# ultralytics/yolov5

Measured on NVIDIA H100. Metric: images/sec @640 (forward + NMS), higher is better.
Workload: dtype bf16

## Files before the change

### yolov5_b200/csrc/conv_gemm.cu

```cuda
#include <cstdio>
#include <cstdlib>
#include <cstring>
#include <mutex>

#include "../../include/y5b200.h"
#include "common.cuh"
#include "host_util.h"
#include "wgmma.cuh"

namespace y5 {

constexpr int kBlockM = 128;
constexpr int kConsumers = 2;
constexpr int kConsumerThreads = 128 * kConsumers;
constexpr int kThreads = 128 + kConsumerThreads;
constexpr int kMaxStages = 8;
constexpr int kHeadN = 128;

enum AMode { A_LINEAR = 0, A_IM2COL = 1, A_PATCH = 2 };

struct ConvParams {
    int M, N;
    int num_m_tiles;
    int num_m_super, num_n_tiles;
    int kh, kw, c_chunks;
    int block_k;
    int a_mode;
    int Ho, Wo, HoWo, stride, pad_h, pad_w;
    int tw, th, tiles_x, tiles_y;
    int b_grouped;
    int patch_pw;
    int cluster_n;
    uint32_t stg_bytes;
    uint32_t b_sub_bytes;
    float rcp_per_img, rcp_tiles_x, rcp_HoWo, rcp_Wo;
    int a_stages, b_stages;
    uint32_t a_sub_bytes, a_stage_bytes, b_stage_bytes;
    int is_bf16, act;
    const float* bias;
    int bias_n;
    void* out;
    int out_pitch;
    const void* res;
    int res_pitch;
    void* raw;
    void* z;
    int na, no, nc, nx, z_rows, z_row0;
    float det_stride;
    float anchor_wh[8];
};

struct SmemLayout {
    uint32_t off_a, off_b, off_out, off_bias, off_bars, total;
};

__host__ __device__ inline SmemLayout smem_layout(int epi, int no, int bias_n, int a_stages, int b_stages, uint32_t a_bytes,
                                                   uint32_t b_bytes, uint32_t stg_bytes) {
    SmemLayout L;
    uint32_t o = 0;
    L.off_a = o;
    o += a_stages * a_bytes;
    L.off_b = o;
    o += b_stages * b_bytes;
    o = (o + 1023) & ~1023u;
    L.off_out = o;
    if (epi == 1) o += 4 * ((kBlockM * no * 2 + 1023) & ~1023u);
    else o += stg_bytes;
    L.off_bias = o;
    o += ((bias_n + 3) & ~3) * 4;
    o = (o + 7) & ~7u;
    L.off_bars = o;
    o += 4 * kMaxStages * 8;
    L.total = o;
    return L;
}

__device__ __forceinline__ int fdiv(int n, int d, float rd) {
    if (n >= (1 << 23)) return n / d;
    int q = __float2int_rz(__int2float_rz(n) * rd);
    const int r = n - q * d;
    if (r >= d) ++q;
    else if (r < 0) --q;
    return q;
}

template <int BLOCK_N, int EPI, int MT, bool OPT>
__global__ void __launch_bounds__(kThreads, 1)
conv_gemm_kernel(const __grid_constant__ CUtensorMap tmA, const __grid_constant__ CUtensorMap tmB, const ConvParams p) {
    static_assert(MT * BLOCK_N <= 256, "accumulators: at most 128 fp32 registers per consumer thread");
    constexpr int kAcc = BLOCK_N / 2;

    extern __shared__ __align__(1024) uint8_t smem_raw[];
    uint8_t* smem = reinterpret_cast<uint8_t*>((reinterpret_cast<uintptr_t>(smem_raw) + 1023) & ~uintptr_t(1023));
    const SmemLayout L = smem_layout(EPI, p.no, p.bias_n, p.a_stages, p.b_stages, p.a_stage_bytes, p.b_stage_bytes, p.stg_bytes);
    uint8_t* sA = smem + L.off_a;
    uint8_t* sB = smem + L.off_b;
    float* sBias = reinterpret_cast<float*>(smem + L.off_bias);
    uint64_t* a_full = reinterpret_cast<uint64_t*>(smem + L.off_bars);
    uint64_t* a_empty = a_full + kMaxStages;
    uint64_t* b_full = a_empty + kMaxStages;
    uint64_t* b_empty = b_full + kMaxStages;

    const int warp = threadIdx.x >> 5;
    const int lane = threadIdx.x & 31;
    const int csize = OPT ? static_cast<int>(cluster_nctarank()) : 1;
    const uint32_t crank = OPT ? cluster_ctarank() : 0u;

    if (threadIdx.x == 0) {
        tma_prefetch_desc(&tmA);
        tma_prefetch_desc(&tmB);
        for (int s = 0; s < kMaxStages; ++s) {
            mbar_init(&a_full[s], 1);
            mbar_init(&a_empty[s], kConsumers);
            mbar_init(&b_full[s], 1);
            mbar_init(&b_empty[s], kConsumers * csize);
        }
        fence_barrier_init();
    }
    if (threadIdx.x >= 128)
        for (int i = threadIdx.x - 128; i < p.bias_n; i += kConsumerThreads) {
            const float b = i < p.N ? __ldg(p.bias + i) : 0.0f;
            sBias[i] = (EPI == 0 && p.act) ? 0.5f * b : b;
        }
    __syncthreads();
    if (csize > 1) cluster_sync_all();
    griddep_wait();
    griddep_launch_dependents();

    const int nn = p.num_n_tiles;
    const int num_tiles = ((p.num_m_super + csize - 1) / csize) * nn;
    const int tile0 = blockIdx.x / csize, tile_step = gridDim.x / csize;
    const uint32_t row_bytes = p.block_k * 2;
    const bool patch = p.a_mode == A_PATCH;
    const bool wide = OPT && p.patch_pw > 0;
    const int grp = wide ? p.kh * p.kw : (patch ? p.kh : 1);
    const int num_groups = wide ? p.c_chunks : (patch ? p.c_chunks * p.kw : p.kh * p.kw * p.c_chunks);

    if (warp < 4) {
        setmaxnreg_dec<56>();
    }
    if (warp == 0) {
        int as = 0, bs = 0;
        uint32_t aph = 0, bph = 0;
        for (int tile = tile0; tile < num_tiles; tile += tile_step) {
            const int ms = (tile / nn) * csize + static_cast<int>(crank);
            const int n0 = (tile - (tile / nn) * nn) * BLOCK_N;
            int img[MT], y0[MT], x0[MT];
#pragma unroll
            for (int mi = 0; mi < MT; ++mi) {
                const int mt = ms * MT + mi;
                img[mi] = y0[mi] = x0[mi] = 0;
                if (p.a_mode == A_IM2COL) {
                    const int m0 = mt * kBlockM;
                    img[mi] = fdiv(m0, p.HoWo, p.rcp_HoWo);
                    const int rem = m0 - img[mi] * p.HoWo;
                    const int oy = fdiv(rem, p.Wo, p.rcp_Wo);
                    y0[mi] = oy * p.stride - p.pad_h;
                    x0[mi] = (rem - oy * p.Wo) * p.stride - p.pad_w;
                } else if (patch) {
                    const int per_img = p.tiles_x * p.tiles_y;
                    img[mi] = fdiv(mt, per_img, p.rcp_per_img);
                    const int rem = mt - img[mi] * per_img;
                    const int ty = fdiv(rem, p.tiles_x, p.rcp_tiles_x);
                    y0[mi] = ty * p.th - p.pad_h;
                    x0[mi] = (rem - ty * p.tiles_x) * p.tw - p.pad_w;
                }
            }
            auto issue_group = [&](int cc, int s, int r0) {
                mbar_wait(&a_empty[as], aph ^ 1);
// ... 16 lines not shown
                for (int j = 0; j < grp; ++j) {
                    const int r = patch ? j : r0;
                    const int kb = wide ? j * p.c_chunks + cc : (r * p.kw + s) * p.c_chunks + cc;
                    const bool stage_first = !p.b_grouped || j == 0, stage_last = !p.b_grouped || j == grp - 1;
                    if (stage_first) mbar_wait(&b_empty[bs], bph ^ 1);
                    if (elect_one()) {
                        if (stage_first) mbar_arrive_expect_tx(&b_full[bs], p.b_stage_bytes);
                        uint8_t* b_dst = sB + bs * p.b_stage_bytes + (p.b_grouped ? j * p.b_sub_bytes : 0u);
                        if (csize == 1) tma_load_2d(&tmB, &b_full[bs], b_dst, kb * p.block_k, n0);
                        else {
                            const int slice_rows = BLOCK_N / csize;
                            tma_load_2d_mcast(&tmB, &b_full[bs], b_dst + crank * slice_rows * row_bytes, kb * p.block_k,
                                              n0 + static_cast<int>(crank) * slice_rows, static_cast<uint16_t>((1u << csize) - 1u));
                        }
                    }
                    __syncwarp();
                    if (stage_last && ++bs == p.b_stages) { bs = 0; bph ^= 1; }
                }
            };
            if (wide) {
                for (int cc = 0; cc < p.c_chunks; ++cc) issue_group(cc, 0, 0);
            } else if (patch) {
                for (int cc = 0; cc < p.c_chunks; ++cc)
                    for (int s = 0; s < p.kw; ++s) issue_group(cc, s, 0);
            } else {
                for (int r = 0; r < p.kh; ++r)
                    for (int s = 0; s < p.kw; ++s)
                        for (int cc = 0; cc < p.c_chunks; ++cc) issue_group(cc, s, r);
            }
        }
    } else if (warp >= 4) {
    setmaxnreg_inc<224>();
    const int wg = (warp >> 2) - 1;
    const int ct = threadIdx.x - 128;
    const int wrow = wg * 64 + (warp & 3) * 16 + (lane >> 2);
    const int ccol = 2 * (lane & 3);
    const bool signal = (threadIdx.x & 127) == 0;
    const bool bf16 = p.is_bf16 != 0;
    const uint32_t dhi = gmma_desc_hi(row_bytes);
    const uint32_t a_hi = wide ? (dhi & ~0x3FFFu) | (((static_cast<uint32_t>(p.patch_pw) * row_bytes) >> 4) & 0x3FFFu) : dhi;
    const uint32_t a_base = gmma_desc_lo(smem_u32(sA) + (wide ? wg * 8 * p.patch_pw : wg * 64) * row_bytes), b_base = gmma_desc_lo(smem_u32(sB));
    const uint32_t row16 = row_bytes >> 4;
    const uint32_t a_stage16 = p.a_stage_bytes >> 4, b_stage16 = p.b_stage_bytes >> 4, a_sub16 = p.a_sub_bytes >> 4;
    const uint32_t b_sub16 = p.b_sub_bytes >> 4;
    const uint32_t a_shift16 = patch ? (p.tw * row_bytes) >> 4 : 0;
    const int k_steps = p.block_k / 16;
    const int per_img = p.tiles_x * p.tiles_y;
    const int tw_shift = patch ? __ffs(p.tw) - 1 : 0;
    int as = 0, bs = 0, head_set = 0;
    uint32_t aph = 0, bph = 0;
    float acc[MT][kAcc];
#pragma unroll
    for (int mi = 0; mi < MT; ++mi)
#pragma unroll
        for (int i = 0; i < kAcc; ++i) acc[mi][i] = 0.0f;

    for (int tile = tile0; tile < num_tiles; tile += tile_step) {
        const int ms = (tile / nn) * csize + static_cast<int>(crank);
        const int nt = tile - (tile / nn) * nn;
        const int n0 = nt * BLOCK_N;
        for (int g = 0; g < num_groups; ++g) {
            mbar_wait(&a_full[as], aph);
            const uint32_t a_stage_lo = a_base + as * a_stage16;
            uint32_t a_lo = a_stage_lo;
            for (int j = 0; j < grp; ++j) {
                if (wide) {
                    const int tr = j / p.kw, ts = j - tr * p.kw;
                    a_lo = a_stage_lo + (tr * p.patch_pw + ts) * row16;
                }
                const bool stage_first = !p.b_grouped || j == 0, stage_last = !p.b_grouped || j == grp - 1;
                if (stage_first) mbar_wait(&b_full[bs], bph);
                const uint32_t b_lo = b_base + bs * b_stage16 + (p.b_grouped ? j * b_sub16 : 0u);
#pragma unroll
                for (int mi = 0; mi < MT; ++mi) fence_regs(acc[mi]);
                wgmma_fence();
#pragma unroll
                for (int k = 0; k < 4; ++k) {
                    if (k < k_steps) {
                        const uint32_t scale_d = (g | j | k) != 0 ? 1u : 0u;
#pragma unroll
                        for (int mi = 0; mi < MT; ++mi) {
                            const uint64_t da = gmma_desc(a_lo + mi * a_sub16 + 2 * k, a_hi), db = gmma_desc(b_lo + 2 * k, dhi);
                            if (bf16) Wgmma<BLOCK_N>::template run<true, 0, 0>(acc[mi], da, db, scale_d);
                            else Wgmma<BLOCK_N>::template run<false, 0, 0>(acc[mi], da, db, scale_d);
                        }
                    }
                }
                wgmma_commit();
                wgmma_wait<0>();
#pragma unroll
                for (int mi = 0; mi < MT; ++mi) fence_regs(acc[mi]);
                if (stage_last) {
                    if (signal) {
                        if (csize == 1) mbar_arrive(&b_empty[bs]);
                        else
                            for (int r = 0; r < csize; ++r) mbar_arrive_cluster(mapa_u32(&b_empty[bs], static_cast<uint32_t>(r)));
                    }
                    if (++bs == p.b_stages) { bs = 0; bph ^= 1; }
                }
                a_lo += a_shift16;
            }
            if (signal) mbar_arrive(&a_empty[as]);
            if (++as == p.a_stages) { as = 0; aph ^= 1; }
        }

        if (EPI == 0) {
            const bool staged = OPT && p.stg_bytes != 0;
            const uint32_t stg_pitch = BLOCK_N * 2 + 16;
            uint8_t* stg = smem + L.off_out + wg * 64 * stg_pitch;
#pragma unroll
            for (int mi = 0; mi < MT; ++mi) {
                const int mt = ms * MT + mi;
                int img = 0, oy0 = 0, ox0 = 0;
                if (patch) {
                    img = fdiv(mt, per_img, p.rcp_per_img);
                    const int rem = mt - img * per_img;
                    const int tyi = fdiv(rem, p.tiles_x, p.rcp_tiles_x);
                    oy0 = tyi * p.th;
                    ox0 = (rem - tyi * p.tiles_x) * p.tw;
                }
                auto pixel_of = [&](int row) -> long long {
                    if (patch) {
                        const int oy = oy0 + (row >> tw_shift), ox = ox0 + (row & ((1 << tw_shift) - 1));
                        return (mt < p.num_m_tiles && oy < p.Ho && ox < p.Wo) ? static_cast<long long>(img) * p.HoWo + oy * p.Wo + ox : -1;
                    }
                    const long long m = static_cast<long long>(mt) * kBlockM + row;
                    return m < p.M ? m : -1;
                };
#pragma unroll
                for (int h = 0; h < 2; ++h) {
                    const int row = wrow + 8 * h;
                    const long long gpix = pixel_of(row);
                    if (gpix < 0 && !staged) continue;
                    uint16_t* op = reinterpret_cast<uint16_t*>(p.out) + gpix * p.out_pitch + n0 + ccol;
                    const uint16_t* rp = (p.res && gpix >= 0) ? reinterpret_cast<const uint16_t*>(p.res) + gpix * p.res_pitch + n0 + ccol : nullptr;
                    uint8_t* sp = stg + (row - wg * 64) * stg_pitch + ccol * 2;
#pragma unroll
                    for (int j = 0; j < BLOCK_N / 8; ++j) {
                        if (n0 + 8 * j >= p.N) continue;
                        const float2 b = *reinterpret_cast<const float2*>(sBias + n0 + 8 * j + ccol);
                        const float a0 = acc[mi][4 * j + 2 * h], a1 = acc[mi][4 * j + 2 * h + 1];
                        float f0, f1;
                        if (p.act) {
                            f0 = silu_from_half(fmaf(a0, 0.5f, b.x));
                            f1 = silu_from_half(fmaf(a1, 0.5f, b.y));
                        } else {
                            f0 = a0 + b.x;
                            f1 = a1 + b.y;
                        }
                        if (rp) {
                            const float2 t = unpack2(*reinterpret_cast<const uint32_t*>(rp + 8 * j), bf16);
                            f0 += t.x;
                            f1 += t.y;
                        }
                        if (staged) *reinterpret_cast<uint32_t*>(sp + 16 * j) = pack2(f0, f1, bf16);
                        else *reinterpret_cast<uint32_t*>(op + 8 * j) = pack2(f0, f1, bf16);
                    }
                }
                if (staged) {
                    named_bar_sync(2 + wg, 128);
                    constexpr int kSeg = BLOCK_N / 8;
                    for (int i = threadIdx.x & 127; i < 64 * kSeg; i += 128) {
                        const int lrow = i / kSeg, c = i - lrow * kSeg;
                        const long long gpix = pixel_of(wg * 64 + lrow);
                        if (gpix >= 0 && n0 + 8 * c < p.N)
                            *reinterpret_cast<uint4*>(reinterpret_cast<uint16_t*>(p.out) + gpix * p.out_pitch + n0 + 8 * c) =
                                *reinterpret_cast<const uint4*>(stg + lrow * stg_pitch + c * 16);
                    }
                    named_bar_sync(2 + wg, 128);
                }
            }
        } else {
            const uint32_t blk = (kBlockM * p.no * 2 + 1023) & ~1023u;
            const int set = head_set;
            head_set ^= 1;
            uint16_t* stage_raw = reinterpret_cast<uint16_t*>(smem + L.off_out + (2 * set) * blk);
            uint16_t* stage_z = reinterpret_cast<uint16_t*>(smem + L.off_out + (2 * set + 1) * blk);
            const int no = p.no;
            const int a = nt;
            const float aw = p.anchor_wh[a * 2], ah = p.anchor_wh[a * 2 + 1];
            const int m0 = ms * kBlockM;
            const int rows_here = min(kBlockM, p.M - m0);
#pragma unroll
            for (int h = 0; h < 2; ++h) {
                const int row = wrow + 8 * h;
                const int m = m0 + row;
                int gx = 0, gy = 0;
                if (m < p.M) { const int pix = m - fdiv(m, p.HoWo, p.rcp_HoWo) * p.HoWo; gy = fdiv(pix, p.nx, p.rcp_Wo); gx = pix - gy * p.nx; }
                const float fgx = static_cast<float>(gx) - 0.5f, fgy = static_cast<float>(gy) - 0.5f;
#pragma unroll
                for (int j = 0; j < BLOCK_N / 8; ++j) {
#pragma unroll
                    for (int e = 0; e < 2; ++e) {
                        const int o = 8 * j + ccol + e;
                        if (o >= no) continue;
                        const float x = acc[0][4 * j + 2 * h + e] + sBias[n0 + o];
                        float d = x;
                        if (o < 5 + p.nc) {
                            const float sg = sigmoid_f(x);
                            if (o == 0) d = (sg * 2.0f + fgx) * p.det_stride;
                            else if (o == 1) d = (sg * 2.0f + fgy) * p.det_stride;
                            else if (o == 2) { const float u = sg * 2.0f; d = u * u * aw; }
                            else if (o == 3) { const float u = sg * 2.0f; d = u * u * ah; }
                            else d = sg;
                        }
                        stage_raw[row * no + o] = pack1(x, bf16);
                        stage_z[row * no + o] = pack1(d, bf16);
                    }
                }
            }
            named_bar_sync(1, kConsumerThreads);
            const int b_lo = fdiv(m0, p.HoWo, p.rcp_HoWo), b_hi = fdiv(m0 + rows_here - 1, p.HoWo, p.rcp_HoWo);
            for (int b = b_lo; b <= b_hi; ++b) {
                const int r_lo = max(b * p.HoWo - m0, 0), r_hi = min((b + 1) * p.HoWo - m0, rows_here);
                const int pix_lo = m0 + r_lo - b * p.HoWo;
                const int n_el = (r_hi - r_lo) * no;
#pragma unroll
                for (int which = 0; which < 2; ++which) {
                    const long long dst_el = which == 0
                        ? ((static_cast<long long>(b) * p.na + a) * p.HoWo + pix_lo) * no
                        : (static_cast<long long>(b) * p.z_rows + p.z_row0 + static_cast<long long>(a) * p.HoWo + pix_lo) * no;
                    uint16_t* dst = reinterpret_cast<uint16_t*>(which == 0 ? p.raw : p.z) + dst_el;
                    const uint16_t* src = (which == 0 ? stage_raw : stage_z) + r_lo * no;
                    if ((((reinterpret_cast<uintptr_t>(dst) | reinterpret_cast<uintptr_t>(src)) & 15) == 0) && (n_el & 7) == 0) {
                        const uint4* s4 = reinterpret_cast<const uint4*>(src);
                        uint4* d4 = reinterpret_cast<uint4*>(dst);
                        for (int i = ct; i < n_el / 8; i += kConsumerThreads) d4[i] = s4[i];
                    } else {
                        for (int i = ct; i < n_el; i += kConsumerThreads) dst[i] = src[i];
                    }
                }
            }
        }
    }
    }
    if (csize > 1) cluster_sync_all();
}

__global__ void conv_direct_kernel(const uint16_t* __restrict__ in, long long xs, long long ys, long long ns, int B, int H,
                                   int W, int Cin, const uint16_t* __restrict__ w, int cin_pad, const float* __restrict__ bias,
                                   uint16_t* out, int out_pitch, int Cout, const uint16_t* res, int res_pitch, int kh, int kw,
                                   int stride, int pad_h, int pad_w, int Ho, int Wo, int act, int bf16) {
    const long long idx = static_cast<long long>(blockIdx.x) * blockDim.x + threadIdx.x;
    const long long total = static_cast<long long>(B) * Ho * Wo * Cout;
    if (idx >= total) return;
    const int n = static_cast<int>(idx % Cout);
    const long long m = idx / Cout;
    const int ox = static_cast<int>(m % Wo);
    const int oy = static_cast<int>((m / Wo) % Ho);
    const int b = static_cast<int>(m / (static_cast<long long>(Wo) * Ho));
    float acc = 0.0f;
    for (int r = 0; r < kh; ++r) {
        const int iy = oy * stride - pad_h + r;
        if (iy < 0 || iy >= H) continue;
        for (int s = 0; s < kw; ++s) {
            const int ix = ox * stride - pad_w + s;
            if (ix < 0 || ix >= W) continue;
            const uint16_t* ip = in + b * ns + iy * ys + ix * xs;
            const uint16_t* wp = w + (static_cast<long long>(n) * kh * kw + r * kw + s) * cin_pad;
            for (int c = 0; c < Cin; ++c) acc += unpack1(ip[c], bf16) * unpack1(wp[c], bf16);
        }
    }
    float x = acc + bias[n];
    if (act) x = x / (1.0f + expf(-x));
    if (res) x += unpack1(res[m * res_pitch + n], bf16);
    out[m * out_pitch + n] = pack1(x, bf16);
}

}

using namespace y5;

namespace {

int pick_block_k(int in_c) {
    return in_c > 16 ? 64 : 16;
}

void pick_tile(int out_c, int64_t m_tiles, int* block_n, int* mt) {
    const int64_t sms = sm_count();
    if (out_c <= 32) { *block_n = 32; *mt = 4; return; }
    if (out_c <= 64) { *block_n = 64; *mt = 2; return; }
    if (out_c <= 128) {
        *block_n = 128;
        *mt = ((m_tiles + 1) / 2) >= sms ? 2 : 1;
        return;
    }
    const int64_t tiles256 = m_tiles * ((out_c + 255) / 256);
    *block_n = (tiles256 >= 2 * sms && (out_c % 256 == 0 || out_c > 384)) ? 256 : 128;
    *mt = 1;
}

int pick_block_n(int out_c, int64_t m_rows) {
    int bn, mt;
    pick_tile(out_c, m_rows > 0 ? (m_rows + kBlockM - 1) / kBlockM : 1, &bn, &mt);
    return bn;
}

template <int BN, int EPI, int MT, bool OPT>
cudaError_t launch_conv(const CUtensorMap& a, const CUtensorMap& b, const ConvParams& p, int grid, int cluster, uint32_t smem,
                        cudaStream_t st) {
    const cudaError_t attr_err = ensure_dyn_smem(reinterpret_cast<const void*>(conv_gemm_kernel<BN, EPI, MT, OPT>), 227 * 1024);
    if (attr_err != cudaSuccess) return attr_err;
    count_launch();
    if (cluster == 1) return launch_pdl(conv_gemm_kernel<BN, EPI, MT, OPT>, dim3(grid), dim3(kThreads), smem, st, a, b, p);
    static const bool pdl = [] { const char* e = getenv("Y5_PDL"); return !(e && e[0] == '0'); }();
    cudaLaunchConfig_t cfg{};
    cfg.gridDim = dim3(grid);
    cfg.blockDim = dim3(kThreads);
    cfg.dynamicSmemBytes = smem;
    cfg.stream = st;
    cudaLaunchAttribute attr[2];
    attr[0].id = cudaLaunchAttributeClusterDimension;
    attr[0].val.clusterDim.x = cluster;
    attr[0].val.clusterDim.y = 1;
    attr[0].val.clusterDim.z = 1;
    attr[1].id = cudaLaunchAttributeProgrammaticStreamSerialization;
    attr[1].val.programmaticStreamSerializationAllowed = 1;
    cfg.attrs = attr;
    cfg.numAttrs = pdl ? 2 : 1;
    return cudaLaunchKernelEx(&cfg, conv_gemm_kernel<BN, EPI, MT, OPT>, a, b, p);
}

struct PlanCommon {
    CUtensorMap tmA, tmB;
    ConvParams p;
    int block_n, epi, mt, grid, cluster;
    uint32_t smem_bytes;
};

int finish_plan(PlanCommon& pc, int block_n, int epi, int mt, int cluster = 1) {
    ConvParams& p = pc.p;
    p.cluster_n = cluster;
    p.a_stage_bytes = mt * p.a_sub_bytes;
    if (p.patch_pw > 0) p.a_stage_bytes = static_cast<uint32_t>(p.th + p.kh - 1) * p.patch_pw * p.block_k * 2;
    p.num_m_super = (p.num_m_tiles + mt - 1) / mt;
    p.num_n_tiles = epi == 1 ? p.na : (p.N + block_n - 1) / block_n;
    p.bias_n = p.num_n_tiles * block_n;
    const uint32_t budget = 225 * 1024 - 1024;
    const bool patch = p.a_mode == A_PATCH;
    int a_st = 0, b_st = 0;
    if (!patch) {
        for (int s = kMaxStages; s >= 2; --s)
            if (smem_layout(epi, p.no, p.bias_n, s, s, p.a_stage_bytes, p.b_stage_bytes, p.stg_bytes).total <= budget) { a_st = b_st = s; break; }
    } else {
        const int b_min = p.b_grouped ? 2 : 3, b_max = p.b_grouped ? 4 : kMaxStages;
        for (int a = 3; a >= 2 && !a_st; --a)
            for (int b = b_max; b >= b_min; --b)
                if (smem_layout(epi, p.no, p.bias_n, a, b, p.a_stage_bytes, p.b_stage_bytes, p.stg_bytes).total <= budget) { a_st = a; b_st = b; break; }
    }
    if (a_st < 2 || b_st < 2) return set_error(Y5_E_UNSUPPORTED, "conv tile does not fit shared memory (block_n %d a %u b %u)", block_n,
                                                p.a_stage_bytes, p.b_stage_bytes);
    p.a_stages = a_st;
    p.b_stages = b_st;
    pc.smem_bytes = smem_layout(epi, p.no, p.bias_n, a_st, b_st, p.a_stage_bytes, p.b_stage_bytes, p.stg_bytes).total + 1024;
    pc.block_n = block_n;
    pc.epi = epi;
    pc.mt = mt;
    pc.cluster = cluster;
    const long long tiles = static_cast<long long>((p.num_m_super + cluster - 1) / cluster) * p.num_n_tiles;
    const int max_clusters = sm_count() / cluster;
    pc.grid = static_cast<int>(tiles < max_clusters ? tiles : max_clusters) * cluster;
    return 0;
}

int run_plan(const PlanCommon& pc, cudaStream_t st) {
    cudaError_t e = cudaErrorInvalidValue;
    const bool opt = pc.cluster > 1 || pc.p.patch_pw > 0 || pc.p.stg_bytes > 0;
    const int key = (opt ? 100000 : 0) + pc.epi * 10000 + pc.block_n * 10 + pc.mt;
    switch (key) {
        case 324: e = launch_conv<32, 0, 4, false>(pc.tmA, pc.tmB, pc.p, pc.grid, pc.cluster, pc.smem_bytes, st); break;
        case 642: e = launch_conv<64, 0, 2, false>(pc.tmA, pc.tmB, pc.p, pc.grid, pc.cluster, pc.smem_bytes, st); break;
        case 1281: e = launch_conv<128, 0, 1, false>(pc.tmA, pc.tmB, pc.p, pc.grid, pc.cluster, pc.smem_bytes, st); break;
        case 1282: e = launch_conv<128, 0, 2, false>(pc.tmA, pc.tmB, pc.p, pc.grid, pc.cluster, pc.smem_bytes, st); break;
        case 2561: e = launch_conv<256, 0, 1, false>(pc.tmA, pc.tmB, pc.p, pc.grid, pc.cluster, pc.smem_bytes, st); break;
        case 11281: e = launch_conv<kHeadN, 1, 1, false>(pc.tmA, pc.tmB, pc.p, pc.grid, pc.cluster, pc.smem_bytes, st); break;
        case 100324: e = launch_conv<32, 0, 4, true>(pc.tmA, pc.tmB, pc.p, pc.grid, pc.cluster, pc.smem_bytes, st); break;
        case 100642: e = launch_conv<64, 0, 2, true>(pc.tmA, pc.tmB, pc.p, pc.grid, pc.cluster, pc.smem_bytes, st); break;
        case 101281: e = launch_conv<128, 0, 1, true>(pc.tmA, pc.tmB, pc.p, pc.grid, pc.cluster, pc.smem_bytes, st); break;
        case 101282: e = launch_conv<128, 0, 2, true>(pc.tmA, pc.tmB, pc.p, pc.grid, pc.cluster, pc.smem_bytes, st); break;
        case 102561: e = launch_conv<256, 0, 1, true>(pc.tmA, pc.tmB, pc.p, pc.grid, pc.cluster, pc.smem_bytes, st); break;
        default: return set_error(Y5_E_UNSUPPORTED, "conv: no kernel for block_n %d mt %d epi %d", pc.block_n, pc.mt, pc.epi);
    }
    if (e != cudaSuccess) return set_error(int(e), "conv_gemm launch failed: %s", cudaGetErrorString(e));
    return 0;
}

bool aligned16(const void* p) { return (reinterpret_cast<uintptr_t>(p) & 15) == 0; }

struct Geo {
    int kh, kw, pad_h, pad_w, Ho, Wo;
    long long xs, ys, ns;
};
Geo geometry(const y5_conv_desc* d) {
    Geo g;
    g.kh = d->ksize;
    g.kw = d->kw ? d->kw : d->ksize;
    g.pad_h = d->pad;
    g.pad_w = d->kw ? d->pad_w : d->pad;
    g.xs = d->in_x_stride ? d->in_x_stride : d->in_pitch;
    g.ys = d->in_y_stride ? d->in_y_stride : static_cast<long long>(d->in_w) * g.xs;
    g.ns = d->in_n_stride ? d->in_n_stride : static_cast<long long>(d->in_h) * g.ys;
    g.Ho = (d->in_h + 2 * g.pad_h - g.kh) / d->stride + 1;
    g.Wo = (d->in_w + 2 * g.pad_w - g.kw) / d->stride + 1;
    return g;
}

}

struct y5_conv_plan {
    PlanCommon pc;
};
struct y5_detect_plan {
    PlanCommon pc;
};

// ... 21 lines not shown
        pw > kw)
        return set_error(Y5_E_UNSUPPORTED, "conv: kernel %dx%d stride %d pad %d,%d unsupported", d->ksize, kw, d->stride, d->pad, pw);
    return 0;
}

extern "C" Y5_API int y5_conv_plan_create(const y5_conv_desc* d, y5_conv_plan** out) {
    if (!out) return set_error(Y5_E_INVALID, "conv: null plan out");
    *out = nullptr;
    if (int e = validate_conv(d)) return e;
    const Geo g = geometry(d);
    if (g.Ho <= 0 || g.Wo <= 0) return set_error(Y5_E_INVALID, "conv: empty output");
    const int64_t M64 = static_cast<int64_t>(d->batch) * g.Ho * g.Wo;
    if (M64 > 0x7fffffff - 256) return set_error(Y5_E_UNSUPPORTED, "conv: more than 2^31 output pixels");
    const int bk = d->block_k ? d->block_k : pick_block_k(d->in_c);
    if (bk != 16 && bk != 32 && bk != 64) return set_error(Y5_E_INVALID, "conv: block_k must be 16/32/64");
    const bool plain = g.kh == 1 && g.kw == 1 && d->stride == 1 && g.pad_h == 0 && g.pad_w == 0 && !d->in_x_stride && !d->in_y_stride &&
                       !d->in_n_stride;
    int best_tw = 0;
    double best_eff = 0.0;
    if (d->stride == 1 && !plain) {
        for (int tw = 8; tw <= 128; tw <<= 1) {
            const int th = 128 / tw;
            const double eff = (double)g.Wo * g.Ho / ((double)((g.Wo + tw - 1) / tw * tw) * ((g.Ho + th - 1) / th * th));
            if (eff > best_eff + 1e-9) { best_eff = eff; best_tw = tw; }
        }
    }
    int a_mode_sel;
    if (plain) a_mode_sel = A_LINEAR;
    else if (d->a_mode == 2 && d->stride != 1) return set_error(Y5_E_INVALID, "conv: patch mode needs stride 1");
    else if (d->a_mode == 2 || (d->a_mode == 0 && d->stride == 1 && best_eff >= 0.75)) a_mode_sel = A_PATCH;
    else a_mode_sel = A_IM2COL;

    int bn = d->block_n, mt_sel = 0, cl_sel = 1;
    {
        int bn_auto = 0;
        pick_tile(d->out_c, (M64 + kBlockM - 1) / kBlockM, &bn_auto, &mt_sel);
        if (!bn) bn = bn_auto;
        else {
            mt_sel = bn < 128 ? 128 / bn : ((d->reserved & 2) && bn == 128 ? 2 : 1);
            cl_sel = (d->reserved >> 8) > 1 ? (d->reserved >> 8) : 1;
            if (d->reserved & 4) cl_sel = 2;
            if (cl_sel != 1 && cl_sel != 2 && cl_sel != 4) return set_error(Y5_E_INVALID, "conv: cluster size must be 1, 2 or 4");
        }
    }
    if (bn != 32 && bn != 64 && bn != 128 && bn != 256) return set_error(Y5_E_INVALID, "conv: block_n must be 32/64/128/256");
    auto* plan = new y5_conv_plan();
    PlanCommon& pc = plan->pc;
    std::memset(&pc.p, 0, sizeof(pc.p));
    ConvParams& p = pc.p;
    p.M = static_cast<int>(M64);
    p.N = d->out_c;
    p.kh = g.kh; p.kw = g.kw;
    p.Ho = g.Ho; p.Wo = g.Wo; p.HoWo = g.Ho * g.Wo;
    p.rcp_HoWo = 1.0f / static_cast<float>(p.HoWo);
    p.rcp_Wo = 1.0f / static_cast<float>(p.Wo);
    p.stride = d->stride;
    p.pad_h = g.pad_h; p.pad_w = g.pad_w;
    p.is_bf16 = d->dtype == Y5_BF16;
    p.act = d->act;
    p.bias = d->bias;
    p.out = d->out;
    p.out_pitch = d->out_pitch;
    p.res = d->residual;
    p.res_pitch = d->res_pitch;
    p.block_k = bk;
    p.c_chunks = (d->in_c + bk - 1) / bk;
    const int row_bytes = bk * 2;
    p.b_sub_bytes = bn * row_bytes;
    p.b_stage_bytes = p.b_sub_bytes;
// ... 21 lines not shown
            const double eff8 = (double)g.Wo * g.Ho / ((double)tx8 * 8 * ty16 * 16);
            if ((d->reserved & 128) && !(d->reserved & 32) && row_bytes == 128 && g.kw > 1 && (mt_sel == 1 || (mt_sel == 2 && tx8 % 2 == 0)) &&
                eff8 >= best_eff - 1e-9) {
                p.tw = 8;
                p.th = 16;
                p.patch_pw = 8 * mt_sel + 8;
            }
        }
        if (!p.patch_pw && g.kh > 1 && bn <= 128) {
            p.b_grouped = 1;
            p.b_stage_bytes = g.kh * p.b_sub_bytes;
        }
        p.tiles_x = (g.Wo + p.tw - 1) / p.tw;
        p.tiles_y = (g.Ho + p.th - 1) / p.th;
        p.rcp_tiles_x = 1.0f / static_cast<float>(p.tiles_x);
        p.rcp_per_img = 1.0f / static_cast<float>(p.tiles_x * p.tiles_y);
        p.num_m_tiles = d->batch * p.tiles_x * p.tiles_y;
        p.a_sub_bytes = p.patch_pw ? 8 * row_bytes : (p.th + g.kh - 1) * p.tw * row_bytes;
        cuuint64_t dims[4] = {(cuuint64_t)d->in_c, (cuuint64_t)d->in_w, (cuuint64_t)d->in_h, (cuuint64_t)d->batch};
        cuuint64_t str[3] = {(cuuint64_t)g.xs * 2, (cuuint64_t)g.ys * 2, (cuuint64_t)g.ns * 2};
        cuuint32_t box[4] = {(cuuint32_t)bk, (cuuint32_t)(p.patch_pw ? p.patch_pw : p.tw), (cuuint32_t)(p.th + g.kh - 1), 1};
        e = encode_tiled(&pc.tmA, d->dtype, d->in, 4, dims, str, box, sw, "A patch");
    }
    if (e) { delete plan; return e; }
    const uint64_t ktot = static_cast<uint64_t>(p.kh) * p.kw * p.c_chunks * bk;
    {
        cuuint64_t dims[2] = {ktot, (cuuint64_t)d->out_c};
        cuuint64_t str[1] = {ktot * 2};
        cuuint32_t box[2] = {(cuuint32_t)bk, (cuuint32_t)(bn / cl_sel)};
        e = encode_tiled(&pc.tmB, d->dtype, d->weight, 2, dims, str, box, sw, "B");
    }
    if (e) { delete plan; return e; }
    p.stg_bytes = ((d->reserved & 8) && !(d->reserved & 16)) ? static_cast<uint32_t>(kConsumers * 64 * (bn * 2 + 16)) : 0u;
    int e2 = finish_plan(pc, bn, 0, mt_sel, cl_sel);
    if (e2 && p.stg_bytes) {
        p.stg_bytes = 0;
        e2 = finish_plan(pc, bn, 0, mt_sel, cl_sel);
    }
    if (e2) { delete plan; return e2; }
    *out = plan;
    return 0;
}

extern "C" Y5_API int y5_conv_plan_run(const y5_conv_plan* plan, void* stream) {
    if (!plan) return set_error(Y5_E_INVALID, "conv: null plan");
    return run_plan(plan->pc, static_cast<cudaStream_t>(stream));
}
extern "C" Y5_API void y5_conv_plan_destroy(y5_conv_plan* plan) { delete plan; }

extern "C" Y5_API int y5_conv_bn_silu_fwd(const y5_conv_desc* d, void* stream) {
    y5_conv_plan* plan = nullptr;
    if (int e = y5_conv_plan_create(d, &plan)) return e;
    const int e = y5_conv_plan_run(plan, stream);
    y5_conv_plan_destroy(plan);
    return e;
}

extern "C" Y5_API int y5_conv_direct_fwd(const y5_conv_desc* d, void* stream) {
    if (int e = validate_conv(d)) return e;
    const Geo g = geometry(d);
    const int bk = d->block_k ? d->block_k : pick_block_k(d->in_c);
    const int cin_pad = (d->in_c + bk - 1) / bk * bk;
    const long long total = static_cast<long long>(d->batch) * g.Ho * g.Wo * d->out_c;
    const int threads = 256;
    const long long blocks = (total + threads - 1) / threads;
    conv_direct_kernel<<<static_cast<unsigned>(blocks), threads, 0, static_cast<cudaStream_t>(stream)>>>(
// ... 26 lines not shown
    p.N = d->na * kHeadN;
    p.kh = p.kw = 1;
    p.Ho = d->ny; p.Wo = d->nx; p.HoWo = d->ny * d->nx;
    p.rcp_HoWo = 1.0f / static_cast<float>(p.HoWo);
    p.rcp_Wo = 1.0f / static_cast<float>(p.Wo);
    p.stride = 1;
    p.is_bf16 = d->dtype == Y5_BF16;
    p.bias = d->bias;
    p.raw = d->raw;
    p.z = d->z;
    p.na = d->na; p.no = d->no; p.nc = d->nc; p.nx = d->nx;
    p.z_rows = d->z_rows; p.z_row0 = d->z_row0;
    p.det_stride = d->stride;
    for (int i = 0; i < 8; ++i) p.anchor_wh[i] = d->anchor_wh[i];
    p.a_mode = A_LINEAR;
    p.block_k = bk;
    p.c_chunks = (d->in_c + bk - 1) / bk;
    const int row_bytes = bk * 2;
    p.a_sub_bytes = kBlockM * row_bytes;
    p.b_stage_bytes = kHeadN * row_bytes;
    p.num_m_tiles = (p.M + kBlockM - 1) / kBlockM;
    const CUtensorMapSwizzle sw = swizzle_for_row_bytes(row_bytes);
    cuuint64_t dims[2] = {(cuuint64_t)d->in_c, (cuuint64_t)p.M};
    cuuint64_t str[1] = {(cuuint64_t)d->in_pitch * 2};
    cuuint32_t box[2] = {(cuuint32_t)bk, kBlockM};
    int e = encode_tiled(&pc.tmA, d->dtype, d->in, 2, dims, str, box, sw, "head A");
    if (e) { delete plan; return e; }
    const uint64_t ktot = static_cast<uint64_t>(p.c_chunks) * bk;
    cuuint64_t bdims[2] = {ktot, (cuuint64_t)p.N};
    cuuint64_t bstr[1] = {ktot * 2};
    cuuint32_t bbox[2] = {(cuuint32_t)bk, (cuuint32_t)kHeadN};
    e = encode_tiled(&pc.tmB, d->dtype, d->weight, 2, bdims, bstr, bbox, sw, "head B");
    if (e) { delete plan; return e; }
    if (int e2 = finish_plan(pc, kHeadN, 1, 1)) { delete plan; return e2; }
    *out = plan;
    return 0;
}
extern "C" Y5_API int y5_detect_plan_run(const y5_detect_plan* plan, void* stream) {
    if (!plan) return set_error(Y5_E_INVALID, "detect: null plan");
    return run_plan(plan->pc, static_cast<cudaStream_t>(stream));
}
extern "C" Y5_API int y5_detect_plan_run_to(const y5_detect_plan* plan, void* raw, void* z, void* stream) {
    if (!plan || !raw || !z) return set_error(Y5_E_INVALID, "detect: null plan/output");
    PlanCommon pc = plan->pc;
    pc.p.raw = raw;
    pc.p.z = z;
    return run_plan(pc, static_cast<cudaStream_t>(stream));
}
extern "C" Y5_API void y5_detect_plan_destroy(y5_detect_plan* plan) { delete plan; }
```

Baseline: 2561.

## Add ping-pong consumer warpgroup schedule with deferred wgmma waits

Adds a ping-pong mode in which each consumer warpgroup owns a whole 128-row tile and the two warpgroups alternate tiles. An ml_turn barrier pair orders their mainloops so one group's epilogue overlaps the other's MMAs. Wgmma waits are relaxed to wait<1>, so smem stage releases are deferred by one step and the next MMA issue overlaps the previous one. Residual loads are also hoisted ahead of the epilogue math. Ping-pong is auto-selected for some conv shapes and always used for the detect head, which adds ring-advance bookkeeping and ordering risk.

```diff
diff --git a/yolov5_b200/csrc/conv_gemm.cu b/yolov5_b200/csrc/conv_gemm.cu
--- a/yolov5_b200/csrc/conv_gemm.cu
+++ b/yolov5_b200/csrc/conv_gemm.cu
@@ -5,6 +5,7 @@
 
 #include "../../include/y5b200.h"
 #include "common.cuh"
+#include "conv_ring.cuh"
 #include "host_util.h"
 #include "wgmma.cuh"
 
@@ -70,7 +71,7 @@
     o += ((bias_n + 3) & ~3) * 4;
     o = (o + 7) & ~7u;
     L.off_bars = o;
-    o += 4 * kMaxStages * 8;
+    o += (4 * kMaxStages + 2) * 8;
     L.total = o;
     return L;
 }
@@ -84,10 +85,13 @@
     return q;
 }
 
-template <int BLOCK_N, int EPI, int MT, bool OPT>
+template <int BLOCK_N, int EPI, int MT, bool OPT, bool PP>
 __global__ void __launch_bounds__(kThreads, 1)
 conv_gemm_kernel(const __grid_constant__ CUtensorMap tmA, const __grid_constant__ CUtensorMap tmB, const ConvParams p) {
     static_assert(MT * BLOCK_N <= 256, "accumulators: at most 128 fp32 registers per consumer thread");
+    static_assert(!PP || (!OPT && MT * BLOCK_N <= 128), "ping-pong: no optional modes, a whole tile in one warpgroup's registers");
+    static_assert(EPI == 0 || PP, "the detect head runs ping-pong");
+    constexpr int kHalves = PP ? 2 : 1;
     constexpr int kAcc = BLOCK_N / 2;
 
     extern __shared__ __align__(1024) uint8_t smem_raw[];
@@ -100,6 +104,7 @@
     uint64_t* a_empty = a_full + kMaxStages;
     uint64_t* b_full = a_empty + kMaxStages;
     uint64_t* b_empty = b_full + kMaxStages;
+    uint64_t* ml_turn = b_empty + kMaxStages;
 
     const int warp = threadIdx.x >> 5;
     const int lane = threadIdx.x & 31;
@@ -109,12 +114,14 @@
     if (threadIdx.x == 0) {
         tma_prefetch_desc(&tmA);
         tma_prefetch_desc(&tmB);
+        constexpr int kReaders = PP ? 1 : kConsumers;
         for (int s = 0; s < kMaxStages; ++s) {
             mbar_init(&a_full[s], 1);
-            mbar_init(&a_empty[s], kConsumers);
+            mbar_init(&a_empty[s], kReaders);
             mbar_init(&b_full[s], 1);
-            mbar_init(&b_empty[s], kConsumers * csize);
-        }
+            mbar_init(&b_empty[s], kReaders * csize);
+        }
+        for (int i = 0; i < 2; ++i) mbar_init(&ml_turn[i], 1);
         fence_barrier_init();
     }
     if (threadIdx.x >= 128)
@@ -133,8 +140,8 @@
     const uint32_t row_bytes = p.block_k * 2;
     const bool patch = p.a_mode == A_PATCH;
     const bool wide = OPT && p.patch_pw > 0;
-    const int grp = wide ? p.kh * p.kw : (patch ? p.kh : 1);
-    const int num_groups = wide ? p.c_chunks : (patch ? p.c_chunks * p.kw : p.kh * p.kw * p.c_chunks);
+    const KLoop kl = k_loop(p.kh, p.kw, p.c_chunks, patch, wide, p.b_grouped != 0);
+    const int grp = kl.grp, num_groups = kl.groups;
 
     if (warp < 4) {
         setmaxnreg_dec<56>();
@@ -217,14 +224,14 @@
     } else if (warp >= 4) {
     setmaxnreg_inc<224>();
     const int wg = (warp >> 2) - 1;
-    const int ct = threadIdx.x - 128;
-    const int wrow = wg * 64 + (warp & 3) * 16 + (lane >> 2);
+    const int wrow = (warp & 3) * 16 + (lane >> 2);
     const int ccol = 2 * (lane & 3);
     const bool signal = (threadIdx.x & 127) == 0;
     const bool bf16 = p.is_bf16 != 0;
     const uint32_t dhi = gmma_desc_hi(row_bytes);
     const uint32_t a_hi = wide ? (dhi & ~0x3FFFu) | (((static_cast<uint32_t>(p.patch_pw) * row_bytes) >> 4) & 0x3FFFu) : dhi;
-    const uint32_t a_base = gmma_desc_lo(smem_u32(sA) + (wide ? wg * 8 * p.patch_pw : wg * 64) * row_bytes), b_base = gmma_desc_lo(smem_u32(sB));
+    const uint32_t a_base = gmma_desc_lo(smem_u32(sA) + (PP ? 0 : wide ? wg * 8 * p.patch_pw : wg * 64) * row_bytes);
+    const uint32_t b_base = gmma_desc_lo(smem_u32(sB));
     const uint32_t row16 = row_bytes >> 4;
     const uint32_t a_stage16 = p.a_stage_bytes >> 4, b_stage16 = p.b_stage_bytes >> 4, a_sub16 = p.a_sub_bytes >> 4;
     const uint32_t b_sub16 = p.b_sub_bytes >> 4;
@@ -232,18 +239,40 @@
     const int k_steps = p.block_k / 16;
     const int per_img = p.tiles_x * p.tiles_y;
     const int tw_shift = patch ? __ffs(p.tw) - 1 : 0;
-    int as = 0, bs = 0, head_set = 0;
-    uint32_t aph = 0, bph = 0;
-    float acc[MT][kAcc];
+    int as = 0, bs = 0;
+    uint32_t aph = 0, bph = 0, ml_ph = 0;
+    if (PP && wg == 1) {
+        ring_advance(as, aph, num_groups, p.a_stages);
+        ring_advance(bs, bph, kl.b_per_tile, p.b_stages);
+    }
+    float acc[MT][kHalves][kAcc];
 #pragma unroll
     for (int mi = 0; mi < MT; ++mi)
 #pragma unroll
-        for (int i = 0; i < kAcc; ++i) acc[mi][i] = 0.0f;
-
-    for (int tile = tile0; tile < num_tiles; tile += tile_step) {
+        for (int hh = 0; hh < kHalves; ++hh)
+#pragma unroll
+            for (int i = 0; i < kAcc; ++i) acc[mi][hh][i] = 0.0f;
+    auto fence_acc = [&] {
+#pragma unroll
+        for (int mi = 0; mi < MT; ++mi)
+#pragma unroll
+            for (int hh = 0; hh < kHalves; ++hh) fence_regs(acc[mi][hh]);
+    };
+
+    auto release_b = [&](int s) {
+        if (!signal) return;
+        if (csize == 1) mbar_arrive(&b_empty[s]);
+        else
+            for (int r = 0; r < csize; ++r) mbar_arrive_cluster(mapa_u32(&b_empty[s], static_cast<uint32_t>(r)));
+    };
+
+    const int tile_first = tile0 + (PP ? wg * tile_step : 0), tile_stride = PP ? 2 * tile_step : tile_step;
+    for (int tile = tile_first; tile < num_tiles; tile += tile_stride) {
         const int ms = (tile / nn) * csize + static_cast<int>(crank);
         const int nt = tile - (tile / nn) * nn;
         const int n0 = nt * BLOCK_N;
+        if (PP && tile != tile0) { mbar_wait(&ml_turn[wg], ml_ph); ml_ph ^= 1; }
+        int rel_a = -1, rel_b = -1;
         for (int g = 0; g < num_groups; ++g) {
             mbar_wait(&a_full[as], aph);
             const uint32_t a_stage_lo = a_base + as * a_stage16;
@@ -256,37 +285,44 @@
                 const bool stage_first = !p.b_grouped || j == 0, stage_last = !p.b_grouped || j == grp - 1;
                 if (stage_first) mbar_wait(&b_full[bs], bph);
                 const uint32_t b_lo = b_base + bs * b_stage16 + (p.b_grouped ? j * b_sub16 : 0u);
-#pragma unroll
-                for (int mi = 0; mi < MT; ++mi) fence_regs(acc[mi]);
+                fence_acc();
                 wgmma_fence();
 #pragma unroll
                 for (int k = 0; k < 4; ++k) {
                     if (k < k_steps) {
                         const uint32_t scale_d = (g | j | k) != 0 ? 1u : 0u;
-#pragma unroll
-                        for (int mi = 0; mi < MT; ++mi) {
-                            const uint64_t da = gmma_desc(a_lo + mi * a_sub16 + 2 * k, a_hi), db = gmma_desc(b_lo + 2 * k, dhi);
-                            if (bf16) Wgmma<BLOCK_N>::template run<true, 0, 0>(acc[mi], da, db, scale_d);
-                            else Wgmma<BLOCK_N>::template run<false, 0, 0>(acc[mi], da, db, scale_d);
-                        }
+                        const uint64_t db = gmma_desc(b_lo + 2 * k, dhi);
+#pragma unroll
+                        for (int mi = 0; mi < MT; ++mi)
+#pragma unroll
+                            for (int hh = 0; hh < kHalves; ++hh) {
+                                const uint64_t da = gmma_desc(a_lo + mi * a_sub16 + hh * 64 * row16 + 2 * k, a_hi);
+                                if (bf16) Wgmma<BLOCK_N>::template run<true, 0, 0>(acc[mi][hh], da, db, scale_d);
+                                else Wgmma<BLOCK_N>::template run<false, 0, 0>(acc[mi][hh], da, db, scale_d);
+                            }
                     }
                 }
                 wgmma_commit();
-                wgmma_wait<0>();
-#pragma unroll
-                for (int mi = 0; mi < MT; ++mi) fence_regs(acc[mi]);
+                wgmma_wait<1>();
+                if (rel_b >= 0) { release_b(rel_b); rel_b = -1; }
+                if (rel_a >= 0) { if (signal) mbar_arrive(&a_empty[rel_a]); rel_a = -1; }
                 if (stage_last) {
-                    if (signal) {
-                        if (csize == 1) mbar_arrive(&b_empty[bs]);
-                        else
-                            for (int r = 0; r < csize; ++r) mbar_arrive_cluster(mapa_u32(&b_empty[bs], static_cast<uint32_t>(r)));
-                    }
+                    rel_b = bs;
                     if (++bs == p.b_stages) { bs = 0; bph ^= 1; }
                 }
                 a_lo += a_shift16;
             }
-            if (signal) mbar_arrive(&a_empty[as]);
+            rel_a = as;
             if (++as == p.a_stages) { as = 0; aph ^= 1; }
+        }
+        if (PP && signal) mbar_arrive(&ml_turn[wg ^ 1]);
+        wgmma_wait<0>();
+        fence_acc();
+        release_b(rel_b);
+        if (signal) mbar_arrive(&a_empty[rel_a]);
+        if (PP) {
+            ring_advance(as, aph, num_groups, p.a_stages);
+            ring_advance(bs, bph, kl.b_per_tile, p.b_stages);
         }
 
         if (EPI == 0) {
@@ -294,8 +330,11 @@
             const uint32_t stg_pitch = BLOCK_N * 2 + 16;
             uint8_t* stg = smem + L.off_out + wg * 64 * stg_pitch;
 #pragma unroll
-            for (int mi = 0; mi < MT; ++mi) {
+            for (int mi = 0; mi < MT; ++mi)
+#pragma unroll
+            for (int hh = 0; hh < kHalves; ++hh) {
                 const int mt = ms * MT + mi;
+                const int rb = (PP ? hh : wg) * 64;
                 int img = 0, oy0 = 0, ox0 = 0;
                 if (patch) {
                     img = fdiv(mt, per_img, p.rcp_per_img);
@@ -314,17 +353,21 @@
                 };
 #pragma unroll
                 for (int h = 0; h < 2; ++h) {
-                    const int row = wrow + 8 * h;
+                    const int row = rb + wrow + 8 * h;
                     const long long gpix = pixel_of(row);
                     if (gpix < 0 && !staged) continue;
                     uint16_t* op = reinterpret_cast<uint16_t*>(p.out) + gpix * p.out_pitch + n0 + ccol;
                     const uint16_t* rp = (p.res && gpix >= 0) ? reinterpret_cast<const uint16_t*>(p.res) + gpix * p.res_pitch + n0 + ccol : nullptr;
-                    uint8_t* sp = stg + (row - wg * 64) * stg_pitch + ccol * 2;
+                    uint8_t* sp = stg + (row - rb) * stg_pitch + ccol * 2;
+                    uint32_t res[BLOCK_N / 8];
+#pragma unroll
+                    for (int j = 0; j < BLOCK_N / 8; ++j)
+                        res[j] = (rp && n0 + 8 * j < p.N) ? *reinterpret_cast<const uint32_t*>(rp + 8 * j) : 0u;
 #pragma unroll
                     for (int j = 0; j < BLOCK_N / 8; ++j) {
                         if (n0 + 8 * j >= p.N) continue;
                         const float2 b = *reinterpret_cast<const float2*>(sBias + n0 + 8 * j + ccol);
-                        const float a0 = acc[mi][4 * j + 2 * h], a1 = acc[mi][4 * j + 2 * h + 1];
+                        const float a0 = acc[mi][hh][4 * j + 2 * h], a1 = acc[mi][hh][4 * j + 2 * h + 1];
                         float f0, f1;
                         if (p.act) {
                             f0 = silu_from_half(fmaf(a0, 0.5f, b.x));
@@ -334,7 +377,7 @@
                             f1 = a1 + b.y;
                         }
                         if (rp) {
-                            const float2 t = unpack2(*reinterpret_cast<const uint32_t*>(rp + 8 * j), bf16);
+                            const float2 t = unpack2(res[j], bf16);
                             f0 += t.x;
                             f1 += t.y;
                         }
@@ -347,7 +390,7 @@
                     constexpr int kSeg = BLOCK_N / 8;
                     for (int i = threadIdx.x & 127; i < 64 * kSeg; i += 128) {
                         const int lrow = i / kSeg, c = i - lrow * kSeg;
-                        const long long gpix = pixel_of(wg * 64 + lrow);
+                        const long long gpix = pixel_of(rb + lrow);
                         if (gpix >= 0 && n0 + 8 * c < p.N)
                             *reinterpret_cast<uint4*>(reinterpret_cast<uint16_t*>(p.out) + gpix * p.out_pitch + n0 + 8 * c) =
                                 *reinterpret_cast<const uint4*>(stg + lrow * stg_pitch + c * 16);
@@ -357,8 +400,8 @@
             }
         } else {
             const uint32_t blk = (kBlockM * p.no * 2 + 1023) & ~1023u;
-            const int set = head_set;
-            head_set ^= 1;
+            const int set = wg;
+            const int ct = threadIdx.x & 127;
             uint16_t* stage_raw = reinterpret_cast<uint16_t*>(smem + L.off_out + (2 * set) * blk);
             uint16_t* stage_z = reinterpret_cast<uint16_t*>(smem + L.off_out + (2 * set + 1) * blk);
             const int no = p.no;
@@ -367,8 +410,10 @@
             const int m0 = ms * kBlockM;
             const int rows_here = min(kBlockM, p.M - m0);
 #pragma unroll
+            for (int hh = 0; hh < kHalves; ++hh)
+#pragma unroll
             for (int h = 0; h < 2; ++h) {
-                const int row = wrow + 8 * h;
+                const int row = hh * 64 + wrow + 8 * h;
                 const int m = m0 + row;
                 int gx = 0, gy = 0;
                 if (m < p.M) { const int pix = m - fdiv(m, p.HoWo, p.rcp_HoWo) * p.HoWo; gy = fdiv(pix, p.nx, p.rcp_Wo); gx = pix - gy * p.nx; }
@@ -379,7 +424,7 @@
                     for (int e = 0; e < 2; ++e) {
                         const int o = 8 * j + ccol + e;
                         if (o >= no) continue;
-                        const float x = acc[0][4 * j + 2 * h + e] + sBias[n0 + o];
+                        const float x = acc[0][hh][4 * j + 2 * h + e] + sBias[n0 + o];
                         float d = x;
                         if (o < 5 + p.nc) {
                             const float sg = sigmoid_f(x);
@@ -394,7 +439,7 @@
                     }
                 }
             }
-            named_bar_sync(1, kConsumerThreads);
+            named_bar_sync(2 + wg, 128);
             const int b_lo = fdiv(m0, p.HoWo, p.rcp_HoWo), b_hi = fdiv(m0 + rows_here - 1, p.HoWo, p.rcp_HoWo);
             for (int b = b_lo; b <= b_hi; ++b) {
                 const int r_lo = max(b * p.HoWo - m0, 0), r_hi = min((b + 1) * p.HoWo - m0, rows_here);
@@ -410,12 +455,13 @@
                     if ((((reinterpret_cast<uintptr_t>(dst) | reinterpret_cast<uintptr_t>(src)) & 15) == 0) && (n_el & 7) == 0) {
                         const uint4* s4 = reinterpret_cast<const uint4*>(src);
                         uint4* d4 = reinterpret_cast<uint4*>(dst);
-                        for (int i = ct; i < n_el / 8; i += kConsumerThreads) d4[i] = s4[i];
+                        for (int i = ct; i < n_el / 8; i += 128) d4[i] = s4[i];
                     } else {
-                        for (int i = ct; i < n_el; i += kConsumerThreads) dst[i] = src[i];
+                        for (int i = ct; i < n_el; i += 128) dst[i] = src[i];
                     }
                 }
             }
+            named_bar_sync(2 + wg, 128);
         }
     }
     }
@@ -482,13 +528,25 @@
     return bn;
 }
 
-template <int BN, int EPI, int MT, bool OPT>
+bool pick_pingpong(int kh, int kw, int stride, int in_c, int out_c) {
+    if (stride == 1 && kh > 1 && kw > 1) return out_c <= 128;
+    return kh == 1 && kw == 1 && stride == 1 && out_c >= 256 && in_c <= 512;
+}
+
+void pick_tile_pingpong(int out_c, int* block_n, int* mt) {
+    if (out_c <= 32) { *block_n = 32; *mt = 4; return; }
+    if (out_c <= 64) { *block_n = 64; *mt = 2; return; }
+    *block_n = 128;
+    *mt = 1;
+}
+
+template <int BN, int EPI, int MT, bool OPT, bool PP = false>
 cudaError_t launch_conv(const CUtensorMap& a, const CUtensorMap& b, const ConvParams& p, int grid, int cluster, uint32_t smem,
                         cudaStream_t st) {
-    const cudaError_t attr_err = ensure_dyn_smem(reinterpret_cast<const void*>(conv_gemm_kernel<BN, EPI, MT, OPT>), 227 * 1024);
+    const cudaError_t attr_err = ensure_dyn_smem(reinterpret_cast<const void*>(conv_gemm_kernel<BN, EPI, MT, OPT, PP>), 227 * 1024);
     if (attr_err != cudaSuccess) return attr_err;
     count_launch();
-    if (cluster == 1) return launch_pdl(conv_gemm_kernel<BN, EPI, MT, OPT>, dim3(grid), dim3(kThreads), smem, st, a, b, p);
+    if (cluster == 1) return launch_pdl(conv_gemm_kernel<BN, EPI, MT, OPT, PP>, dim3(grid), dim3(kThreads), smem, st, a, b, p);
     static const bool pdl = [] { const char* e = getenv("Y5_PDL"); return !(e && e[0] == '0'); }();
     cudaLaunchConfig_t cfg{};
     cfg.gridDim = dim3(grid);
@@ -504,13 +562,14 @@
     attr[1].val.programmaticStreamSerializationAllowed = 1;
     cfg.attrs = attr;
     cfg.numAttrs = pdl ? 2 : 1;
-    return cudaLaunchKernelEx(&cfg, conv_gemm_kernel<BN, EPI, MT, OPT>, a, b, p);
+    return cudaLaunchKernelEx(&cfg, conv_gemm_kernel<BN, EPI, MT, OPT, PP>, a, b, p);
 }
 
 struct PlanCommon {
     CUtensorMap tmA, tmB;
     ConvParams p;
     int block_n, epi, mt, grid, cluster;
+    bool pp;
     uint32_t smem_bytes;
 };
 
@@ -552,21 +611,26 @@
 int run_plan(const PlanCommon& pc, cudaStream_t st) {
     cudaError_t e = cudaErrorInvalidValue;
     const bool opt = pc.cluster > 1 || pc.p.patch_pw > 0 || pc.p.stg_bytes > 0;
-    const int key = (opt ? 100000 : 0) + pc.epi * 10000 + pc.block_n * 10 + pc.mt;
+    const int key = (pc.pp ? 200000 : opt ? 100000 : 0) + pc.epi * 10000 + pc.block_n * 10 + pc.mt;
+#define Y5_CONV(BN, EPI, MT, OPT, PP) e = launch_conv<BN, EPI, MT, OPT, PP>(pc.tmA, pc.tmB, pc.p, pc.grid, pc.cluster, pc.smem_bytes, st); break
     switch (key) {
-        case 324: e = launch_conv<32, 0, 4, false>(pc.tmA, pc.tmB, pc.p, pc.grid, pc.cluster, pc.smem_bytes, st); break;
-        case 642: e = launch_conv<64, 0, 2, false>(pc.tmA, pc.tmB, pc.p, pc.grid, pc.cluster, pc.smem_bytes, st); break;
-        case 1281: e = launch_conv<128, 0, 1, false>(pc.tmA, pc.tmB, pc.p, pc.grid, pc.cluster, pc.smem_bytes, st); break;
-        case 1282: e = launch_conv<128, 0, 2, false>(pc.tmA, pc.tmB, pc.p, pc.grid, pc.cluster, pc.smem_bytes, st); break;
-        case 2561: e = launch_conv<256, 0, 1, false>(pc.tmA, pc.tmB, pc.p, pc.grid, pc.cluster, pc.smem_bytes, st); break;
-        case 11281: e = launch_conv<kHeadN, 1, 1, false>(pc.tmA, pc.tmB, pc.p, pc.grid, pc.cluster, pc.smem_bytes, st); break;
-        case 100324: e = launch_conv<32, 0, 4, true>(pc.tmA, pc.tmB, pc.p, pc.grid, pc.cluster, pc.smem_bytes, st); break;
-        case 100642: e = launch_conv<64, 0, 2, true>(pc.tmA, pc.tmB, pc.p, pc.grid, pc.cluster, pc.smem_bytes, st); break;
-        case 101281: e = launch_conv<128, 0, 1, true>(pc.tmA, pc.tmB, pc.p, pc.grid, pc.cluster, pc.smem_bytes, st); break;
-        case 101282: e = launch_conv<128, 0, 2, true>(pc.tmA, pc.tmB, pc.p, pc.grid, pc.cluster, pc.smem_bytes, st); break;
-        case 102561: e = launch_conv<256, 0, 1, true>(pc.tmA, pc.tmB, pc.p, pc.grid, pc.cluster, pc.smem_bytes, st); break;
+        case 324: Y5_CONV(32, 0, 4, false, false);
+        case 642: Y5_CONV(64, 0, 2, false, false);
+        case 1281: Y5_CONV(128, 0, 1, false, false);
+        case 1282: Y5_CONV(128, 0, 2, false, false);
+        case 2561: Y5_CONV(256, 0, 1, false, false);
+        case 100324: Y5_CONV(32, 0, 4, true, false);
+        case 100642: Y5_CONV(64, 0, 2, true, false);
+        case 101281: Y5_CONV(128, 0, 1, true, false);
+        case 101282: Y5_CONV(128, 0, 2, true, false);
+        case 102561: Y5_CONV(256, 0, 1, true, false);
+        case 200324: Y5_CONV(32, 0, 4, false, true);
+        case 200642: Y5_CONV(64, 0, 2, false, true);
+        case 201281: Y5_CONV(128, 0, 1, false, true);
+        case 211281: Y5_CONV(kHeadN, 1, 1, false, true);
         default: return set_error(Y5_E_UNSUPPORTED, "conv: no kernel for block_n %d mt %d epi %d", pc.block_n, pc.mt, pc.epi);
     }
+#undef Y5_CONV
     if (e != cudaSuccess) return set_error(int(e), "conv_gemm launch failed: %s", cudaGetErrorString(e));
     return 0;
 }
@@ -654,9 +718,11 @@
     else a_mode_sel = A_IM2COL;
 
     int bn = d->block_n, mt_sel = 0, cl_sel = 1;
+    const bool pp = !d->block_n && !d->reserved && pick_pingpong(g.kh, g.kw, d->stride, d->in_c, d->out_c);
     {
         int bn_auto = 0;
-        pick_tile(d->out_c, (M64 + kBlockM - 1) / kBlockM, &bn_auto, &mt_sel);
+        if (pp) pick_tile_pingpong(d->out_c, &bn_auto, &mt_sel);
+        else pick_tile(d->out_c, (M64 + kBlockM - 1) / kBlockM, &bn_auto, &mt_sel);
         if (!bn) bn = bn_auto;
         else {
             mt_sel = bn < 128 ? 128 / bn : ((d->reserved & 2) && bn == 128 ? 2 : 1);
@@ -744,6 +810,7 @@
     }
     if (e) { delete plan; return e; }
     p.stg_bytes = ((d->reserved & 8) && !(d->reserved & 16)) ? static_cast<uint32_t>(kConsumers * 64 * (bn * 2 + 16)) : 0u;
+    pc.pp = pp;
     int e2 = finish_plan(pc, bn, 0, mt_sel, cl_sel);
     if (e2 && p.stg_bytes) {
         p.stg_bytes = 0;
@@ -836,6 +903,7 @@
     cuuint32_t bbox[2] = {(cuuint32_t)bk, (cuuint32_t)kHeadN};
     e = encode_tiled(&pc.tmB, d->dtype, d->weight, 2, bdims, bstr, bbox, sw, "head B");
     if (e) { delete plan; return e; }
+    pc.pp = true;
     if (int e2 = finish_plan(pc, kHeadN, 1, 1)) { delete plan; return e2; }
     *out = plan;
     return 0;
diff --git a/yolov5_b200/csrc/conv_ring.cuh b/yolov5_b200/csrc/conv_ring.cuh
--- /dev/null
+++ b/yolov5_b200/csrc/conv_ring.cuh
@@ -0,0 +1,24 @@
+#pragma once
+#include <stdint.h>
+
+namespace y5 {
+
+struct KLoop {
+    int grp, groups, b_per_tile;
+};
+
+__host__ __device__ inline KLoop k_loop(int kh, int kw, int c_chunks, bool patch, bool wide, bool b_grouped) {
+    KLoop k;
+    k.grp = wide ? kh * kw : (patch ? kh : 1);
+    k.groups = wide ? c_chunks : (patch ? c_chunks * kw : kh * kw * c_chunks);
+    k.b_per_tile = b_grouped ? k.groups : k.groups * k.grp;
+    return k;
+}
+
+__host__ __device__ inline void ring_advance(int& stage, uint32_t& phase, int count, int stages) {
+    stage += count;
+    phase ^= static_cast<uint32_t>(stage / stages) & 1u;
+    stage %= stages;
+}
+
+}
```

Result: faster. 2817 (median of 6 runs) (+10.0%).
